# virajmehta/vae-training

Measured on AMD Instinct MI355X. Metric: ELBO train-step samples/sec, higher is better.
Workload: dtype f32; 1 GPU; M: linear-padding dd3 pad9 (D=12) L=20 linear enc/dec -tdv eps=-1 lr=1e-3 (seed_linpadding_expts.sh:1); batch_per_gpu=65536, global_batch=65536, data_dim=12, latent_dim=20, params=533, parallelism=dp1, grad_exchange=none, launch=direct library call x2395 steps (arguments marshalled once), input_batches=48

## Files before the change

### vae_training_amd/csrc/linear_moments.hip

```cpp
#include <stdlib.h>

#include <type_traits>

#include "comm_dev.h"
#include "rng_dev.h"
#include "vaek_internal.h"

namespace vaek {

using f32x4 = __attribute__((ext_vector_type(4))) float;
using d2 = __attribute__((ext_vector_type(2))) double;
typedef __attribute__((address_space(3))) void lds_void_t;
typedef const __attribute__((address_space(1))) void glb_void_t;

constexpr int LNT = 512, LNW = LNT / 64;
constexpr int kLinMaxPersist = 64;
constexpr int kLinCarry = 2, kLinSlots = kLinMaxPersist + kLinCarry;
struct LinWindow { int first, count; };
struct LinWindows { LinWindow stream, reduce, update; };
constexpr LinWindows lin_windows(int K, int j) {
    const int s0 = kLinMaxPersist * j, s1 = s0 + kLinMaxPersist < K ? s0 + kLinMaxPersist : K;
    const bool last = s1 == K;
    const int r0 = s0 >= 1 ? s0 - 1 : 0, u0 = s0 >= 2 ? s0 - 2 : 0;
    return LinWindows{{s0, s1 - s0}, {r0, (last ? K : s1 - 1) - r0}, {u0, (last ? K : s1 - 2) - u0}};
}
constexpr int lin_launches(int K) { return (K + kLinMaxPersist - 1) / kLinMaxPersist; }
constexpr bool lin_windows_ok(int K) {
    int s = 0, r = 0, u = 0;
    for (int j = 0; j < lin_launches(K); ++j) {
        const LinWindows w = lin_windows(K, j);
        if (w.stream.first != s || w.reduce.first != r || w.update.first != u) return false;
        if (w.stream.count < 1 || w.stream.count > kLinMaxPersist || w.reduce.count < 1 || w.update.count < 1) return false;
        s += w.stream.count; r += w.reduce.count; u += w.update.count;
        if (r > s || u > r || s - w.update.first > kLinSlots) return false;
    }
    return s == K && r == K && u == K;
}
static_assert(lin_windows_ok(1) && lin_windows_ok(2) && lin_windows_ok(64) && lin_windows_ok(65) && lin_windows_ok(66) && lin_windows_ok(128) &&
              lin_windows_ok(129) && lin_windows_ok(130) && lin_windows_ok(960), "launch windows of a vaek_train_steps call");
static_assert(lin_windows(64, 0).update.count == 64 && lin_windows(130, 1).update.first == 62 && lin_windows(130, 1).reduce.first == 63 &&
              lin_windows(130, 2).update.count == 4, "launch windows of a vaek_train_steps call");
constexpr int kLinReduceSets = 1;
constexpr int kLinReduceWgs = 24;

constexpr int kLinCommBanks = 4;
struct LinComm { unsigned long long* peer[kMaxWorld]; int world, rank, ng2; };

constexpr int kLinShards = 8, kLinShardStride = 32;
struct LinPtrs { const float* x[64]; const float* z1[64]; const float* z2[64]; };
struct LinArgs {
    int has_update, n_reduce, n_stream;
    int B, D, L, ntiles, T;
    const float* x; const float* z1; const float* z2; float* partial_out;
    const float* partial_in; double* M_out;
    const double* M_in;
    int persistent, n_steps, sets;
    int n_red, n_str, slot_upd, slot_red, slot_str;
    int d_red, d_str;
    float* partial_base; double* M_base;
    unsigned* cnt_stream; unsigned* cnt_reduce; unsigned* status;
    float* params; float* grads; float* m; float* v; int32_t* step_dev; float lr;
    float inv_bt, eps_cli, rows, rows_over_bt; int off_eps, P;
    float* loss_hist; long long loss_hist_cap;
    int stagger;
    LinComm comm;
};

#ifndef VAEK_LIN_ABL
#define VAEK_LIN_ABL 0
#endif
#ifdef VAEK_LIN_STAMPS
#ifdef VAEK_LIN_FOUR_BLOCK_TU
static __device__ unsigned long long* g_lin_stamp_buf = nullptr;
#else
__device__ unsigned long long* g_lin_stamp_buf = nullptr;
#endif
int lin_stamps_four(unsigned long long* buf);
#define LIN_STAMP(i)                                                                                         \
    do {                                                                                                     \
        if (VAEK_LIN_STAMPS == 2) break;          \
        __builtin_amdgcn_sched_barrier(0);                                                                   \
        unsigned long long _t;                                                                               \
        unsigned long long _r;                                                                               \
        asm volatile("s_waitcnt vmcnt(0) lgkmcnt(0)\n\ts_memtime %0\n\ts_memrealtime %1\n\ts_waitcnt lgkmcnt(0)" : "=s"(_t), "=s"(_r)::"memory"); \
        if (g_lin_stamp_buf && threadIdx.x == 0) { g_lin_stamp_buf[i] = _t; g_lin_stamp_buf[16 + (i)] = _r; } \
        __builtin_amdgcn_sched_barrier(0);                                                                   \
    } while (0)
#define LIN_NOW(v)                                                                                           \
    do {                                                                                                     \
        __builtin_amdgcn_sched_barrier(0);                                                                   \
        if (VAEK_LIN_STAMPS == 2) asm volatile("s_memrealtime %0\n\ts_waitcnt lgkmcnt(0)" : "=s"(v)::"memory");             \
        else asm volatile("s_waitcnt vmcnt(0) lgkmcnt(0)\n\ts_memrealtime %0\n\ts_waitcnt lgkmcnt(0)" : "=s"(v)::"memory"); \
        __builtin_amdgcn_sched_barrier(0);                                                                   \
    } while (0)
#define LIN_NOWQ(v)                                     \
    do {                                                                                                     \
        __builtin_amdgcn_sched_barrier(0);                                                                   \
        asm volatile("s_memrealtime %0\n\ts_waitcnt lgkmcnt(0)" : "=s"(v)::"memory");                        \
        __builtin_amdgcn_sched_barrier(0);                                                                   \
    } while (0)
#define LIN_PUT(i, v) do { if (g_lin_stamp_buf && threadIdx.x == 0) g_lin_stamp_buf[i] = (v); } while (0)
#define LIN_PUTMAX(i, v) do { if (g_lin_stamp_buf && threadIdx.x == 0) atomicMax(&g_lin_stamp_buf[i], (v)); } while (0)
#else
#define LIN_STAMP(i) do {} while (0)
#define LIN_NOW(v) do {} while (0)
#define LIN_NOWQ(v) do {} while (0)
#define LIN_PUT(i, v) do {} while (0)
#define LIN_PUTMAX(i, v) do {} while (0)
#endif

__device__ __forceinline__ void lin_glds16(const void* gsrc, void* lds_wave_base) {
    __builtin_amdgcn_global_load_lds((glb_void_t*)gsrc, (lds_void_t*)lds_wave_base, 16, 0, 0);
}
template <int N> __device__ __forceinline__ void lin_wait_vmcnt() { asm volatile("s_waitcnt vmcnt(%0)" ::"n"(N) : "memory"); }
__device__ __forceinline__ void lin_barrier() { asm volatile("s_waitcnt lgkmcnt(0)\n\ts_barrier" ::: "memory"); }
__device__ __forceinline__ void lin_wait_vmcnt_upto(int n) {
    switch (n) {
        case 1: lin_wait_vmcnt<1>(); break;   case 2: lin_wait_vmcnt<2>(); break;   case 3: lin_wait_vmcnt<3>(); break;
        case 4: lin_wait_vmcnt<4>(); break;   case 5: lin_wait_vmcnt<5>(); break;   case 6: lin_wait_vmcnt<6>(); break;
        case 7: lin_wait_vmcnt<7>(); break;   case 8: lin_wait_vmcnt<8>(); break;   case 9: lin_wait_vmcnt<9>(); break;
        case 10: lin_wait_vmcnt<10>(); break; case 11: lin_wait_vmcnt<11>(); break; case 12: lin_wait_vmcnt<12>(); break;
        case 13: lin_wait_vmcnt<13>(); break; case 14: lin_wait_vmcnt<14>(); break; case 15: lin_wait_vmcnt<15>(); break;
        case 16: lin_wait_vmcnt<16>(); break; case 17: lin_wait_vmcnt<17>(); break; case 18: lin_wait_vmcnt<18>(); break;
        case 19: lin_wait_vmcnt<19>(); break; case 20: lin_wait_vmcnt<20>(); break;
        default: lin_wait_vmcnt<0>(); break;
    }
}

__device__ __host__ constexpr int lin_blk(int NB, int b1, int b2) { return b1 * NB - b1 * (b1 - 1) / 2 + (b2 - b1); }

__device__ __forceinline__ void st_sc1(float* p, float v) { __hip_atomic_store(p, v, __ATOMIC_RELAXED, __HIP_MEMORY_SCOPE_AGENT); }
__device__ __forceinline__ void st_sc1(double* p, double v) { __hip_atomic_store(p, v, __ATOMIC_RELAXED, __HIP_MEMORY_SCOPE_AGENT); }
__device__ __forceinline__ float ld_sc1(const float* p) { return __hip_atomic_load(p, __ATOMIC_RELAXED, __HIP_MEMORY_SCOPE_AGENT); }
__device__ __forceinline__ double ld_sc1(const double* p) { return __hip_atomic_load(p, __ATOMIC_RELAXED, __HIP_MEMORY_SCOPE_AGENT); }

__device__ __forceinline__ void lin_wait_count(const unsigned* cnt, unsigned target, unsigned* status, unsigned tag) {
    if (threadIdx.x == 0) {
        unsigned spins = 0, seen;
        while ((seen = __hip_atomic_load(cnt, __ATOMIC_RELAXED, __HIP_MEMORY_SCOPE_AGENT)) < target) {
            __builtin_amdgcn_s_sleep(16);
            if ((++spins & 1023u) == 0) {
                if (__hip_atomic_load(status, __ATOMIC_RELAXED, __HIP_MEMORY_SCOPE_AGENT)) break;
                if (spins > (1u << 21)) {
                    unsigned expect = 0;
                    __hip_atomic_compare_exchange_strong(status, &expect, 0x80000000u | tag | (seen & 0xffffu), __ATOMIC_RELAXED,
                                                         __ATOMIC_RELAXED, __HIP_MEMORY_SCOPE_AGENT);
                    break;
                }
            }
        }
    }
    __syncthreads();
}

__device__ __forceinline__ void lin_wait_shards(const unsigned* cnt, unsigned target, unsigned* status, unsigned tag) {
    if (threadIdx.x == 0) {
        unsigned spins = 0, seen;
        for (;;) {
            unsigned v[kLinShards];
#pragma unroll
            for (int k = 0; k < kLinShards; ++k) v[k] = __hip_atomic_load(cnt + k * kLinShardStride, __ATOMIC_RELAXED, __HIP_MEMORY_SCOPE_AGENT);
            seen = 0;
#pragma unroll
            for (int k = 0; k < kLinShards; ++k) seen += v[k];
            if (seen >= target) break;
            __builtin_amdgcn_s_sleep(4);
            if ((++spins & 1023u) == 0) {
                if (__hip_atomic_load(status, __ATOMIC_RELAXED, __HIP_MEMORY_SCOPE_AGENT)) break;
                if (spins > (1u << 21)) {
                    unsigned expect = 0;
                    __hip_atomic_compare_exchange_strong(status, &expect, 0x80000000u | tag | (seen & 0xffffu), __ATOMIC_RELAXED,
                                                         __ATOMIC_RELAXED, __HIP_MEMORY_SCOPE_AGENT);
                    break;
                }
            }
        }
    }
    __syncthreads();
}

__device__ __forceinline__ double lin_sum_over_ranks(const LinComm& c, unsigned epoch, int o, double v, unsigned* status) {
    const unsigned long long bits = (unsigned long long)__double_as_longlong(v), tag = (unsigned long long)epoch << 32;
    const long long bank = (long long)(epoch & (kLinCommBanks - 1)) * c.world * c.ng2;
    for (int p = 0; p < c.world; ++p) {
        unsigned long long* q = c.peer[p] + bank + (long long)c.rank * c.ng2 + 2 * o;
        __hip_atomic_store(q, tag | (bits & 0xffffffffull), __ATOMIC_RELAXED, __HIP_MEMORY_SCOPE_SYSTEM);
        __hip_atomic_store(q + 1, tag | (bits >> 32), __ATOMIC_RELAXED, __HIP_MEMORY_SCOPE_SYSTEM);
    }
    const unsigned long long* own = c.peer[c.rank] + bank + 2 * o;
    double sum = 0.0;
    unsigned spins = 0;
    bool dead = false;
    for (int r = 0; r < c.world; ++r) {
        unsigned long long lo = 0, hi = 0;
// ... 435 lines not shown
            for (int d = 0; d < (DT ? DT : 32); ++d) if (DT || d < D) s += Wdd[l * D + d] * P1[d * NFP + f];
            G[e] = s;
        }
        for (int e = t; e < L * D; e += LNT) {
            const int l = e / D, d = e % D;
            double s = sd[l] * P1[d * NFP + l] + bed[l] * P1[d * NFP + fone];
#pragma unroll
            for (int dd = 0; dd < (DT ? DT : 32); ++dd) if (DT || dd < D) s += Wed[dd * L + l] * P1[d * NFP + L + dd];
            dwd[e] = s;
        }
        }
        __syncthreads();
        LIN_STAMP(4);
        double ssq = 0.0, musq = 0.0, z2r = 0.0, klc = 0.0;
        if constexpr (DT > 0 && LT > 0 && (DT % 2 == 0) && (LT % 2 == 0) && LT * (NFP / 2) <= LNT && LT * DT <= LNT / 2) {
            static_assert(DT * LT + LT + LT * DT + DT + LT + 1 + 3 <= LNT + 64, "wave 0 must own the scalar outputs");
            if (t < 64) {
                constexpr int NS = (LT * DT + 63) / 64, NM = (LT * (DT + 1) + 63) / 64;
                double wa[NS], da[NS], qw[NM], qs[NM], qd[NM], qm[NM];
#pragma unroll
                for (int j = 0; j < NS; ++j) { const int e = min(t + 64 * j, LT * DT - 1); wa[j] = Wdd[e]; da[j] = dwd[e]; }
#pragma unroll
                for (int j = 0; j < NM; ++j) {
                    const int e = min(t + 64 * j, LT * (DT + 1) - 1), l = e / (DT + 1), dd = e % (DT + 1), f = dd < DT ? LT + dd : fone;
                    qw[j] = dd < DT ? Wed[dd * LT + l] : bed[l]; qs[j] = SM[l * NFP + f]; qd[j] = sd[l]; qm[j] = Mf[l * NFP + f];
                }
                const int dq = min(t, DT - 1), lq = min(t, LT - 1);
                const double px = P1[dq * NFP + LT + dq], pz = P1[dq * NFP + LT + DT + dq], po = P1[dq * NFP + fone], bq = bdd[dq];
                const double lvq = lvd[lq], evq = elv[lq];
                __builtin_amdgcn_sched_barrier(0);
#pragma unroll
                for (int j = 0; j < NS; ++j) ssq += t + 64 * j < LT * DT ? wa[j] * da[j] : 0.0;
#pragma unroll
                for (int j = 0; j < NM; ++j) musq += t + 64 * j < LT * (DT + 1) ? qw[j] * (qs[j] - qd[j] * qm[j]) : 0.0;
                if (t < DT) { ssq += -px + sigma * pz + bq * po; z2r = pz; }
                if (t < LT) klc = 1.0 + lvq - evq;
#pragma unroll
                for (int o = 32; o > 0; o >>= 1) {
                    ssq += __shfl_xor(ssq, o, 64); musq += __shfl_xor(musq, o, 64);
                    z2r += __shfl_xor(z2r, o, 64); klc += __shfl_xor(klc, o, 64);
                }
            }
        } else {
        double p_ssq = 0.0, p_musq = 0.0, p_z2r = 0.0, p_klc = 0.0;
        for (int e = t; e < L * D; e += LNT) p_ssq += Wdd[e] * dwd[e];
        if (t < D) {
            p_ssq += -P1[t * NFP + L + t] + sigma * P1[t * NFP + L + D + t] + bdd[t] * P1[t * NFP + fone];
            p_z2r = P1[t * NFP + L + D + t];
        }
        for (int e = t; e < L * (D + 1); e += LNT) {
            const int l = e / (D + 1), dd = e % (D + 1);
            const int f = dd < D ? L + dd : fone;
            const double q = SM[l * NFP + f] - sd[l] * Mf[l * NFP + f];
            p_musq += (dd < D ? Wed[dd * L + l] : bed[l]) * q;
        }
        if (t < L) p_klc = 1.0 + lvd[t] - elv[t];
#pragma unroll
        for (int o = 32; o > 0; o >>= 1) {
            p_ssq += __shfl_xor(p_ssq, o, 64); p_musq += __shfl_xor(p_musq, o, 64);
            p_z2r += __shfl_xor(p_z2r, o, 64); p_klc += __shfl_xor(p_klc, o, 64);
        }
        if ((t & 63) == 0) { red[t >> 6] = p_ssq; red[LNW + (t >> 6)] = p_musq; red[2 * LNW + (t >> 6)] = p_z2r; red[3 * LNW + (t >> 6)] = p_klc; }
        __syncthreads();
#pragma unroll
        for (int w = 0; w < LNW; ++w) { ssq += red[w]; musq += red[LNW + w]; z2r += red[2 * LNW + w]; klc += red[3 * LNW + w]; }
        }
        LIN_STAMP(5);
        const double inv_bt = (double)a.inv_bt, rows = (double)a.rows, c0 = inv_var * inv_bt;
        const float bc1 = -expm1f((float)tstep * -0.10536051565782628f), bc2 = -expm1f((float)tstep * -0.0010005003335835335f);
#pragma unroll
        for (int k = 0; k < LKOUT; ++k) {
            const int idx = t + LNT * k;
            double gd = 0.0;
            if (idx < off_be) { const int d = idx / L, l = idx % L; gd = c0 * G[l * NFP + L + d] + (SM[l * NFP + L + d] - sd[l] * Mf[l * NFP + L + d]) * inv_bt; }
            else if (idx < off_wd) { const int l = idx - off_be; gd = c0 * G[l * NFP + fone] + (SM[l * NFP + fone] - sd[l] * Mf[l * NFP + fone]) * inv_bt; }
            else if (idx < off_bd) gd = c0 * dwd[idx - off_wd];
            else if (idx < off_epsp) gd = c0 * P1[(idx - off_bd) * NFP + fone];
            else if (idx < off_epsp + L) {
                const int l = idx - off_epsp;
                gd = 0.5 * sd[l] * c0 * G[l * NFP + l] - 0.5 * (1.0 - elv[l]) * (double)a.rows_over_bt;
            } else if (idx == off_eps) {
                gd = (double)a.eps_cli * (-0.5 * ssq * inv_var + 0.5 * rows * D + 0.5 * sigma * z2r * inv_var) * inv_bt;
            } else if (idx >= P && idx < P + 3) {
                const double dkl = (0.5 * musq - 0.5 * rows * klc) * inv_bt;
                const double mse = (0.5 * ssq * inv_var + 0.5 * rows * D * ((double)kLog2Pi + eps)) * inv_bt;
                gd = idx == P ? dkl + mse : (idx == P + 1 ? dkl : mse);
            }
            const float gf = (float)gd;
            gout[k] = gf;
            if (idx == P && a.loss_hist) a.loss_hist[(long long)(tstep - 1) % a.loss_hist_cap] = gf;
            if (idx < P) adam_apply_f(p[k], gf, m[k], v[k], a.lr, bc1, bc2);
        }
        LIN_STAMP(6);
    }
    __device__ __forceinline__ void store_state(const LinArgs& a, const float (&gout)[LKOUT], int tstep) {
        const int t = threadIdx.x;
#pragma unroll
        for (int k = 0; k < LKOUT; ++k) {
            const int idx = t + LNT * k;
            if (idx < P + kExtra) a.grads[idx] = gout[k];
            if (idx < P) { a.params[idx] = p[k]; a.m[idx] = m[k]; a.v[idx] = v[k]; }
        }
        if (t == 0) a.step_dev[0] = tstep;
    }
};

using d4 = __attribute__((ext_vector_type(4))) double;
template <int CTRL>
__device__ __forceinline__ double lin_dpp_add(double x) {
    const int lo = __builtin_amdgcn_update_dpp(0, __double2loint(x), CTRL, 0xf, 0xf, false);
    const int hi = __builtin_amdgcn_update_dpp(0, __double2hiint(x), CTRL, 0xf, 0xf, false);
    return x + __hiloint2double(hi, lo);
}
__device__ __forceinline__ double lin_wave_sum(double x) {
    x = lin_dpp_add<0xB1>(x);
    x = lin_dpp_add<0x4E>(x);
    x = lin_dpp_add<0x141>(x);
    x = lin_dpp_add<0x140>(x);
    double tot = 0.0;
#pragma unroll
    for (int r = 0; r < 4; ++r)
        tot += __hiloint2double(__builtin_amdgcn_readlane(__double2hiint(x), 16 * r), __builtin_amdgcn_readlane(__double2loint(x), 16 * r));
    return tot;
}
template <bool InLoop = false>
__device__ __forceinline__ double lin_exp(double x) {
    auto c = [](double v) __attribute__((always_inline)) { if constexpr (InLoop) asm volatile("" : "+s"(v)); return v; };
    const double k = rint(x * c(1.4426950408889634));
    double r = fma(-k, c(6.93147180369123816490e-01), x);
    r = fma(-k, c(1.90821492927058770002e-10), r);
    double p = c(1.0 / 6227020800.0);
    p = fma(p, r, c(1.0 / 479001600.0)); p = fma(p, r, c(1.0 / 39916800.0)); p = fma(p, r, c(1.0 / 3628800.0)); p = fma(p, r, c(1.0 / 362880.0));
    p = fma(p, r, c(1.0 / 40320.0)); p = fma(p, r, c(1.0 / 5040.0)); p = fma(p, r, c(1.0 / 720.0)); p = fma(p, r, c(1.0 / 120.0));
    p = fma(p, r, c(1.0 / 24.0)); p = fma(p, r, c(1.0 / 6.0)); p = fma(p, r, 0.5); p = fma(p, r, 1.0); p = fma(p, r, 1.0);
    return ldexp(p, (int)k);
}
__device__ __forceinline__ int lin_m_index(int NB, int r, int c) {
    const int br = r >> 4, bc = c >> 4;
    const int b1 = br <= bc ? br : bc, b2 = br <= bc ? bc : br, i = br <= bc ? (r & 15) : (c & 15), j = br <= bc ? (c & 15) : (r & 15);
    return lin_blk(NB, b1, b2) * 256 + (((i >> 2) * 16 + j) << 2) + (i & 3);
}
template <int NB, int DT, int LT>
struct LinUpdM {
    static constexpr int NFP = 16 * NB;
    static constexpr int KD = DT ? (DT + 3) / 4 : 4;
    static constexpr int RL1 = LT ? (LT > 16 ? (LT - 16 + 3) / 4 : 0) : 4;
    static constexpr int NM = 4 + RL1 + 2 * KD + 1;
    int D, L, P, fone, off_be, off_wd, off_bd, off_epsp, off_eps;
    double *Wed, *Wdd, *bed, *bdd, *sd, *elv, *lvd, *scal, *part, *P1s, *gq;
    float p[LKOUT], m[LKOUT], v[LKOUT];
    int mo[NM];

    static __host__ __device__ constexpr bool shape_ok(int D, int L) { return D <= 16 && L <= 32 && L + 2 * D + 1 <= NFP && NB == 3; }
    static __host__ size_t lds_bytes(int D, int L, int P) {
        return sizeof(double) * ((size_t)2 * D * L + 4 * L + D + 8 + 16 + 16 * NFP + (size_t)(P + kExtra + 7));
    }
    __device__ __forceinline__ void carve(const LinArgs& a, char* smem) {
        D = DT ? DT : a.D; L = LT ? LT : a.L; P = a.P; fone = L + 2 * D; off_eps = a.off_eps;
        off_be = D * L; off_wd = off_be + L; off_bd = off_wd + L * D; off_epsp = off_bd + D;
        Wed = reinterpret_cast<double*>(smem); Wdd = Wed + D * L; bed = Wdd + L * D; bdd = bed + L; sd = bdd + D; elv = sd + L; lvd = elv + L;
        scal = lvd + L; part = scal + 8; P1s = part + 16; gq = P1s + 16 * NFP;
    }
    __device__ __forceinline__ void load_state(const LinArgs& a) {
        const int t = threadIdx.x;
#pragma unroll
        for (int k = 0; k < LKOUT; ++k) {
            const int idx = min(t + LNT * k, P - 1);
            p[k] = a.params[idx]; m[k] = a.m[idx]; v[k] = a.v[idx];
        }
        if (off_eps < 0 && t == 0) { const double e = (double)a.eps_cli; scal[0] = e; scal[1] = lin_exp(0.5 * e); scal[2] = lin_exp(-e); }
        const int lane = t & 63, j = lane & 15, g = lane >> 4, f = min(16 * (t >> 6) + j, NFP - 1);
        int k = 0;
#pragma unroll
        for (int r = 0; r < 4; ++r) mo[k++] = lin_m_index(NB, g + 4 * r, f);
#pragma unroll
        for (int r = 0; r < RL1; ++r) mo[k++] = lin_m_index(NB, min(16 + g + 4 * r, NFP - 1), f);
#pragma unroll
        for (int r = 0; r < KD; ++r) mo[k++] = lin_m_index(NB, min(L + g + 4 * r, NFP - 1), f);
#pragma unroll
        for (int r = 0; r < KD; ++r) mo[k++] = lin_m_index(NB, min(L + D + g + 4 * r, NFP - 1), f);
        mo[k++] = lin_m_index(NB, fone, f);
    }
    __device__ __forceinline__ void fetch_M(const double* M_in, double (&r)[NM]) const {
#pragma unroll
        for (int k = 0; k < NM; ++k) r[k] = ld_sc1(M_in + mo[k]);
    }
    __device__ __forceinline__ void publish_params(const LinArgs& a) {
        const int t = threadIdx.x;
#pragma unroll
        for (int k = 0; k < LKOUT; ++k) {
            const int i = t + LNT * k;
            const double pv = (double)p[k];
            if (i < off_be) Wed[i] = pv;
            else if (i < off_wd) bed[i - off_be] = pv;
            else if (i < off_bd) Wdd[i - off_wd] = pv;
            else if (i < off_epsp) bdd[i - off_bd] = pv;
            else if (i < off_epsp + L || i == off_eps) {
                const bool is_eps = i == off_eps;
                const double e = is_eps ? pv * (double)a.eps_cli : pv, h = lin_exp(0.5 * e);
                if (is_eps) {
                    const double q = h * h;
                    double r = __builtin_amdgcn_rcp(q);
                    r = fma(fma(-q, r, 1.0), r, r); r = fma(fma(-q, r, 1.0), r, r);
                    scal[0] = e; scal[1] = h; scal[2] = r;
                }
                else { sd[i - off_epsp] = h; elv[i - off_epsp] = h * h; lvd[i - off_epsp] = pv; }
            }
        }
    }
    __device__ __forceinline__ void step(const LinArgs& a, int tstep, const double (&mreg)[NM], float (&gout)[LKOUT], const unsigned* next_cnt,
                                         unsigned per_set, const double* M_next, double (&mnext)[NM], bool& have_next) {
        const int t = threadIdx.x, wave = __builtin_amdgcn_readfirstlane(t >> 6), lane = t & 63, j = lane & 15, g = lane >> 4;
        LIN_STAMP(1);
        if (t == 64 * (NB + 2)) scal[4] = (next_cnt && __hip_atomic_load(next_cnt, __ATOMIC_RELAXED, __HIP_MEMORY_SCOPE_AGENT) >= per_set) ? 1.0 : 0.0;
        const double eps = scal[0], sigma = scal[1], inv_var = scal[2], inv_bt = (double)a.inv_bt, c0 = inv_var * inv_bt;
        d4 sm[2], p1;
        double musq_p = 0.0, ssq_p = 0.0, z2r_p = 0.0;
        const int f = 16 * wave + j;
        double awSMr[KD][2], awP1r[4 + (RL1 ? RL1 : 1)];
        auto awSM = [&](int kk, int lt) -> double& { return awSMr[kk][lt]; };
        auto awP1 = [&](int r) -> double& { return awP1r[r]; };
        if (wave < NB) {
#pragma unroll
            for (int kk = 0; kk < KD; ++kk)
#pragma unroll
                for (int lt = 0; lt < 2; ++lt) {
                    const int dd = 4 * kk + g, l = 16 * lt + j;
                    const double w1 = Wed[min(dd, D - 1) * L + min(l, L - 1)];
                    awSM(kk, lt) = (dd < D && l < L && (lt == 0 || RL1 > 0)) ? w1 : 0.0;
                }
#pragma unroll
            for (int r = 0; r < 4 + RL1; ++r) {
                const int l = (r < 4 ? 4 * r : 16 + 4 * (r - 4)) + g;
                const double w = Wdd[min(l, L - 1) * D + min(j, D - 1)];
                awP1(r) = (j < D && l < L) ? w : 0.0;
            }
        }
        __builtin_amdgcn_sched_barrier(0);
        if (wave < NB) {
            const double* Mz = mreg; const double* Mx = mreg + 4 + RL1; const double* Mz2 = Mx + KD; const double Mone = mreg[NM - 1];
#pragma unroll
            for (int lt = 0; lt < 2; ++lt)
#pragma unroll
                for (int r = 0; r < 4; ++r) {
                    const int l = 16 * lt + g + 4 * r;
                    const bool ok = l < L && (lt == 0 || r < RL1);
                    const double sv = sd[min(l, L - 1)], bv = bed[min(l, L - 1)];
                    const double slv = ok ? sv : 0.0, blv = ok ? bv : 0.0;
                    sm[lt][r] = (lt == 0 || r < RL1) ? slv * Mz[lt == 0 ? r : min(4 + r, 3 + RL1)] + blv * Mone : 0.0;
                }
#pragma unroll
            for (int kk = 0; kk < KD; ++kk) {
#pragma unroll
                for (int lt = 0; lt < 2; ++lt) {
                    if (lt == 1 && RL1 == 0) continue;
                    sm[lt] = __builtin_amdgcn_mfma_f64_16x16x4f64(awSM(kk, lt), Mx[kk], sm[lt], 0, 0, 0);
                }
            }
#pragma unroll
            for (int r = 0; r < 4; ++r) {
                const int d = g + 4 * r;
                p1[r] = (r < KD && d < D) ? -Mx[min(r, KD - 1)] + sigma * Mz2[min(r, KD - 1)] + bdd[min(d, D - 1)] * Mone : 0.0;
            }
#pragma unroll
            for (int r = 0; r < 4; ++r) p1 = __builtin_amdgcn_mfma_f64_16x16x4f64(awP1(r), sm[0][r], p1, 0, 0, 0);
#pragma unroll
            for (int r = 0; r < RL1; ++r) p1 = __builtin_amdgcn_mfma_f64_16x16x4f64(awP1(4 + r), sm[1][r], p1, 0, 0, 0);
#pragma unroll
            for (int r = 0; r < 4; ++r) P1s[(g + 4 * r) * NFP + f] = p1[r];
        } else if (wave == NB + 1) {
            const double kl = lane < L ? 1.0 + lvd[min(lane, L - 1)] - elv[min(lane, L - 1)] : 0.0;
            const double tot = lin_wave_sum(kl);
            if (lane == 0) {
                part[12] = tot;
                part[13] = (double)(-expm1f((float)tstep * -0.10536051565782628f)); part[14] = (double)(-expm1f((float)tstep * -0.0010005003335835335f));
            }
        }
        LIN_STAMP(2);
        __syncthreads();
        LIN_STAMP(3);
        have_next = scal[4] != 0.0;
        if (wave < NB) {
            if (have_next) fetch_M(M_next, mnext);
            double awGr[KD][2];
#pragma unroll
            for (int kk = 0; kk < KD; ++kk)
#pragma unroll
                for (int lt = 0; lt < 2; ++lt) {
                    const int dd = 4 * kk + g, l = 16 * lt + j;
                    const double w2 = Wdd[min(l, L - 1) * D + min(dd, D - 1)];
                    awGr[kk][lt] = (l < L && dd < D && (lt == 0 || RL1 > 0)) ? w2 : 0.0;
                }
            double sl[2][4], bl[2][4];
#pragma unroll
            for (int lt = 0; lt < 2; ++lt)
#pragma unroll
                for (int r = 0; r < 4; ++r) {
                    const int l = 16 * lt + g + 4 * r;
                    const bool ok = l < L && (lt == 0 || r < RL1);
                    const double sv = sd[min(l, L - 1)], bv = bed[min(l, L - 1)];
                    sl[lt][r] = ok ? sv : 0.0; bl[lt][r] = ok ? bv : 0.0;
                }
            __builtin_amdgcn_sched_barrier(0);
            d4 G[2];
            G[0] = d4{0.0, 0.0, 0.0, 0.0}; G[1] = d4{0.0, 0.0, 0.0, 0.0};
#pragma unroll
            for (int r = 0; r < KD; ++r) {
#pragma unroll
                for (int lt = 0; lt < 2; ++lt) {
                    if (lt == 1 && RL1 == 0) continue;
                    G[lt] = __builtin_amdgcn_mfma_f64_16x16x4f64(awGr[r][lt], p1[r], G[lt], 0, 0, 0);
                }
            }
            const double* Mz = mreg;
            const bool is_x = f >= L && f < L + D, is_z2 = f >= L + D && f < fone, is_one = f == fone, is_z1 = f < L;
            if (is_x || is_one) {
                const int base = is_x ? (f - L) * L : off_be;
#pragma unroll
                for (int lt = 0; lt < 2; ++lt)
#pragma unroll
                    for (int r = 0; r < 4; ++r) {
                        if (lt == 1 && r >= RL1) continue;
                        const int l = 16 * lt + g + 4 * r;
                        if (l < L) {
                            const double q = sm[lt][r] - sl[lt][r] * Mz[lt == 0 ? r : min(4 + r, 3 + RL1)];
                            gq[base + l] = c0 * G[lt][r] + q * inv_bt;
                            musq_p += (is_x ? Wed[base + l] : bl[lt][r]) * q;
                        }
                    }
            }
            if (is_one) {
#pragma unroll
                for (int r = 0; r < 4; ++r) {
                    const int d = g + 4 * r;
                    if (d < D) { gq[off_bd + d] = c0 * p1[r]; ssq_p += bdd[d] * p1[r]; }
                }
            }
            if (is_z1 && (j & 3) == g) {
                const int lt = f >> 4, r = j >> 2;
                double gll = 0.0;
#pragma unroll
                for (int q2 = 0; q2 < 2; ++q2)
#pragma unroll
                    for (int r2 = 0; r2 < 4; ++r2) gll = (q2 == lt && r2 == r) ? G[q2][r2] : gll;
                gq[off_epsp + f] = 0.5 * sd[f] * c0 * gll - 0.5 * (1.0 - elv[f]) * (double)a.rows_over_bt;
            }
            if (is_x || is_z2) {
                const int d = is_x ? f - L : f - L - D;
                if ((d & 3) == g) {
                    double pd = 0.0;
#pragma unroll
                    for (int r2 = 0; r2 < 4; ++r2) pd = (r2 == (d >> 2)) ? p1[r2] : pd;
                    if (is_x) ssq_p -= pd; else { ssq_p += sigma * pd; z2r_p += pd; }
                }
            }
            musq_p = lin_wave_sum(musq_p); ssq_p = lin_wave_sum(ssq_p); z2r_p = lin_wave_sum(z2r_p);
            if (lane == 0) { part[3 * wave] = ssq_p; part[3 * wave + 1] = musq_p; part[3 * wave + 2] = z2r_p; }
        } else if (wave == NB) {
            d4 C[2];
            double wsum = 0.0, avk[KD], p1l[2][4], p1o[4], dw_sr[2], dw_br[2], dw_wr[KD][2], dw_dr[2][4];
            auto dw_s = [&](int ct) -> double& { return dw_sr[ct]; };
            auto dw_b = [&](int ct) -> double& { return dw_br[ct]; };
            auto dw_w = [&](int kk, int ct) -> double& { return dw_wr[kk][ct]; };
            auto dw_d = [&](int ct, int r) -> double& { return dw_dr[ct][r]; };
#pragma unroll
            for (int ct = 0; ct < 2; ++ct) {
                const int l = 16 * ct + j, lc = min(l, L - 1);
                const double s_l = sd[lc], b_l = bed[lc];
                dw_s(ct) = l < L ? s_l : 0.0; dw_b(ct) = l < L ? b_l : 0.0;
#pragma unroll
                for (int kk = 0; kk < KD; ++kk) {
                    const int dd = 4 * kk + g;
                    const double w = Wed[min(dd, D - 1) * L + lc];
                    dw_w(kk, ct) = (dd < D && l < L) ? w : 0.0;
                }
#pragma unroll
                for (int r = 0; r < 4; ++r) dw_d(ct, r) = Wdd[lc * D + min(g + 4 * r, D - 1)];
            }
#pragma unroll
            for (int kk = 0; kk < KD; ++kk) avk[kk] = P1s[j * NFP + min(L + 4 * kk + g, NFP - 1)];
#pragma unroll
            for (int r = 0; r < 4; ++r) {
                p1o[r] = P1s[(g + 4 * r) * NFP + fone];
#pragma unroll
                for (int ct = 0; ct < 2; ++ct) p1l[ct][r] = P1s[(g + 4 * r) * NFP + min(16 * ct + j, L - 1)];
            }
            __builtin_amdgcn_sched_barrier(0);
#pragma unroll
            for (int ct = 0; ct < 2; ++ct) {
                if (ct == 1 && RL1 == 0) continue;
                const int l = 16 * ct + j;
#pragma unroll
                for (int r = 0; r < 4; ++r) C[ct][r] = dw_s(ct) * p1l[ct][r] + dw_b(ct) * p1o[r];
#pragma unroll
                for (int kk = 0; kk < KD; ++kk) C[ct] = __builtin_amdgcn_mfma_f64_16x16x4f64(avk[kk], dw_w(kk, ct), C[ct], 0, 0, 0);
#pragma unroll
                for (int r = 0; r < 4; ++r) {
                    const int d = g + 4 * r;
                    if (l < L && d < D) { gq[off_wd + l * D + d] = c0 * C[ct][r]; wsum += dw_d(ct, r) * C[ct][r]; }
                }
            }
            wsum = lin_wave_sum(wsum);
            if (lane == 0) part[9] = wsum;
        }
        LIN_STAMP(4);
        __syncthreads();
        LIN_STAMP(5);
        const double rows = (double)a.rows;
        const float bc1 = (float)part[13], bc2 = (float)part[14];
#pragma unroll
        for (int k = 0; k < LKOUT; ++k) {
            const int idx = t + LNT * k;
            if (LNT * k >= P + 3) break;
            double gd = 0.0;
            if (idx < P && idx != off_eps) gd = gq[idx];
            else if (idx == off_eps || (idx >= P && idx < P + 3)) {
                const double ssq = part[0] + part[3] + part[6] + part[9], musq = part[1] + part[4] + part[7], z2r = part[2] + part[5] + part[8], klc = part[12];
                if (idx == off_eps) gd = (double)a.eps_cli * (-0.5 * ssq * inv_var + 0.5 * rows * D + 0.5 * sigma * z2r * inv_var) * inv_bt;
                else {
                    const double dkl = (0.5 * musq - 0.5 * rows * klc) * inv_bt;
                    const double mse = (0.5 * ssq * inv_var + 0.5 * rows * D * ((double)kLog2Pi + eps)) * inv_bt;
                    gd = idx == P ? dkl + mse : (idx == P + 1 ? dkl : mse);
                }
            }
            const float gf = (float)gd;
            gout[k] = gf;
            if (idx == P && a.loss_hist) a.loss_hist[(long long)(tstep - 1) % a.loss_hist_cap] = gf;
            if (idx < P) adam_apply_f(p[k], gf, m[k], v[k], a.lr, bc1, bc2);
        }
        LIN_STAMP(6);
    }
    __device__ __forceinline__ void store_state(const LinArgs& a, const float (&gout)[LKOUT], int tstep) {
        const int t = threadIdx.x;
#pragma unroll
        for (int k = 0; k < LKOUT; ++k) {
            const int idx = t + LNT * k;
            if (idx < P + kExtra) a.grads[idx] = gout[k];
            if (idx < P) { a.params[idx] = p[k]; a.m[idx] = m[k]; a.v[idx] = v[k]; }
        }
        if (t == 0) a.step_dev[0] = tstep;
    }
};

template <int NB, int DT, int LT>
struct LinUpdMG {
    static constexpr int NFP = 16 * NB;
    static constexpr int KD = DT ? (DT + 3) / 4 : (NB == 3 ? 4 : 8);
    static constexpr int RL1 = LT ? (LT > 16 ? (LT - 16 + 3) / 4 : 0) : 4;
    static constexpr int NM = 4 + RL1 + 2 * KD + 1;
    static constexpr int PT = KD > 4 ? 2 : 1;
    static constexpr int NPART = NB == 3 ? 16 : 20;
    static constexpr bool PREFETCH = NB == 3;
    int D, L, P, fone, off_be, off_wd, off_bd, off_epsp, off_eps;
    double *Wed, *Wdd, *bed, *bdd, *sd, *elv, *lvd, *scal, *part, *P1s, *gq;
    float* pmv;
    __device__ __forceinline__ float& pk(int k) const { return pmv[k * LNT + threadIdx.x]; }
    __device__ __forceinline__ float& mk(int k) const { return pmv[(LKOUT + k) * LNT + threadIdx.x]; }
    __device__ __forceinline__ float& vk(int k) const { return pmv[(2 * LKOUT + k) * LNT + threadIdx.x]; }
    int* mos;

    static __host__ __device__ constexpr bool shape_ok(int D, int L) {
        return NB == 3 ? D <= 16 && L <= 32 && L + 2 * D + 1 <= NFP : NB == 4 && L <= 32 && L + 2 * D + 1 <= NFP && D <= 4 * KD;
    }
    static __host__ size_t lds_bytes(int D, int L, int P) {
        return sizeof(double) * ((size_t)2 * D * L + 4 * L + D + 8 + NPART + 16 * PT * NFP + (size_t)(P + kExtra + 7)) + sizeof(int) * NM * 64 * NB + sizeof(float) * 3 * LKOUT * LNT;
    }
    __device__ __forceinline__ void carve(const LinArgs& a, char* smem) {
        D = DT ? DT : a.D; L = LT ? LT : a.L; P = a.P; fone = L + 2 * D; off_eps = a.off_eps;
        off_be = D * L; off_wd = off_be + L; off_bd = off_wd + L * D; off_epsp = off_bd + D;
        Wed = reinterpret_cast<double*>(smem); Wdd = Wed + D * L; bed = Wdd + L * D; bdd = bed + L; sd = bdd + D; elv = sd + L; lvd = elv + L;
        scal = lvd + L; part = scal + 8; P1s = part + NPART; gq = P1s + 16 * PT * NFP; mos = reinterpret_cast<int*>(gq + P + kExtra + 7);
        pmv = reinterpret_cast<float*>(smem + sizeof(double) * (size_t)(gq + P + kExtra + 7 - Wed) + sizeof(int) * NM * 64 * NB);
    }
    __device__ __forceinline__ void load_state(const LinArgs& a) {
        const int t = threadIdx.x;
#pragma unroll
        for (int k = 0; k < LKOUT; ++k) {
            const int idx = min(t + LNT * k, P - 1);
            pk(k) = a.params[idx]; mk(k) = a.m[idx]; vk(k) = a.v[idx];
        }
        if (off_eps < 0 && t == 0) { const double e = (double)a.eps_cli; scal[0] = e; scal[1] = lin_exp<true>(0.5 * e); scal[2] = lin_exp<true>(-e); }
        if (t < 64 * NB) {
            const int lane = t & 63, j = lane & 15, g = lane >> 4, f = 16 * (t >> 6) + j;
            int k = 0;
            auto put = [&](int row) { mos[(k++) * 64 * NB + t] = lin_m_index(NB, row, f); };
#pragma unroll
            for (int r = 0; r < 4; ++r) put(g + 4 * r);
#pragma unroll
            for (int r = 0; r < RL1; ++r) put(min(16 + g + 4 * r, NFP - 1));
#pragma unroll
            for (int r = 0; r < KD; ++r) put(min(L + g + 4 * r, NFP - 1));
#pragma unroll
            for (int r = 0; r < KD; ++r) put(min(L + D + g + 4 * r, NFP - 1));
            put(fone);
        }
    }
    __device__ __forceinline__ void fetch_M(const double* M_in, double (&r)[NM]) const {
        const int* mt = mos + threadIdx.x;
        int o[NM];
#pragma unroll
        for (int k = 0; k < NM; ++k) o[k] = mt[k * 64 * NB];
#pragma unroll
        for (int k = 0; k < NM; ++k) r[k] = ld_sc1(M_in + o[k]);
    }
    __device__ __forceinline__ void publish_params(const LinArgs& a) {
        int t = threadIdx.x;
        if constexpr (NB == 4) asm volatile("" : "+v"(t));
#pragma unroll
        for (int k = 0; k < LKOUT; ++k) {
            const int i = t + LNT * k;
            const double pv = (double)pk(k);
            if (i < off_be) Wed[i] = pv;
            else if (i < off_wd) bed[i - off_be] = pv;
            else if (i < off_bd) Wdd[i - off_wd] = pv;
            else if (i < off_epsp) bdd[i - off_bd] = pv;
            else if (i < off_epsp + L || i == off_eps) {
                const bool is_eps = i == off_eps;
                const double e = is_eps ? pv * (double)a.eps_cli : pv, h = lin_exp<true>(0.5 * e);
                if (is_eps) {
                    const double q = h * h;
                    double r = __builtin_amdgcn_rcp(q);
                    r = fma(fma(-q, r, 1.0), r, r); r = fma(fma(-q, r, 1.0), r, r);
                    scal[0] = e; scal[1] = h; scal[2] = r;
                }
                else { sd[i - off_epsp] = h; elv[i - off_epsp] = h * h; lvd[i - off_epsp] = pv; }
            }
        }
    }
    __device__ __forceinline__ void step(const LinArgs& a, int tstep, const double (&mreg)[NM], float (&gout)[LKOUT], const unsigned* next_cnt,
                                         unsigned per_set, const double* M_next, double (&mnext)[NM], bool& have_next) {
        int t = threadIdx.x;
        if constexpr (NB == 4) asm volatile("" : "+v"(t));
        const int wave = __builtin_amdgcn_readfirstlane(t >> 6), lane = t & 63, j = lane & 15, g = lane >> 4;
        LIN_STAMP(1);
        if (PREFETCH && t == 64 * (NB + 2)) scal[4] = (next_cnt && __hip_atomic_load(next_cnt, __ATOMIC_RELAXED, __HIP_MEMORY_SCOPE_AGENT) >= per_set) ? 1.0 : 0.0;
        const double eps = scal[0], sigma = scal[1], inv_var = scal[2], inv_bt = (double)a.inv_bt, c0 = inv_var * inv_bt;
        d4 sm[2], p1;
        [[maybe_unused]] d4 p1b;
        auto p1row = [&](int r) -> double { return r < 4 ? p1[r & 3] : p1b[r & 3]; };
        double musq_p = 0.0, ssq_p = 0.0, z2r_p = 0.0;
        const int f = 16 * wave + j;
        double awSMr[KD][2], awP1r[PT][4 + (RL1 ? RL1 : 1)];
        auto awSM = [&](int kk, int lt) -> double& { return awSMr[kk][lt]; };
        auto awP1 = [&](int r) -> double& { return awP1r[0][r]; };
        if (wave < NB) {
#pragma unroll
            for (int kk = 0; kk < KD; ++kk)
#pragma unroll
                for (int lt = 0; lt < 2; ++lt) {
                    const int dd = 4 * kk + g, l = 16 * lt + j;
                    const double w1 = Wed[min(dd, D - 1) * L + min(l, L - 1)];
                    awSM(kk, lt) = (dd < D && l < L && (lt == 0 || RL1 > 0)) ? w1 : 0.0;
                }
#pragma unroll
            for (int r = 0; r < 4 + RL1; ++r) {
                const int l = (r < 4 ? 4 * r : 16 + 4 * (r - 4)) + g;
                const double w = Wdd[min(l, L - 1) * D + min(j, D - 1)];
                awP1(r) = (j < D && l < L) ? w : 0.0;
            }
        }
        __builtin_amdgcn_sched_barrier(0);
        if (wave < NB) {
            const double* Mz = mreg; const double* Mx = mreg + 4 + RL1; const double* Mz2 = Mx + KD; const double Mone = mreg[NM - 1];
#pragma unroll
            for (int lt = 0; lt < 2; ++lt)
#pragma unroll
                for (int r = 0; r < 4; ++r) {
                    const int l = 16 * lt + g + 4 * r;
                    const bool ok = l < L && (lt == 0 || r < RL1);
                    const double sv = sd[min(l, L - 1)], bv = bed[min(l, L - 1)];
                    const double slv = ok ? sv : 0.0, blv = ok ? bv : 0.0;
                    sm[lt][r] = (lt == 0 || r < RL1) ? slv * Mz[lt == 0 ? r : min(4 + r, 3 + RL1)] + blv * Mone : 0.0;
                }
#pragma unroll
            for (int kk = 0; kk < KD; ++kk) {
#pragma unroll
                for (int lt = 0; lt < 2; ++lt) {
                    if (lt == 1 && RL1 == 0) continue;
                    sm[lt] = __builtin_amdgcn_mfma_f64_16x16x4f64(awSM(kk, lt), Mx[kk], sm[lt], 0, 0, 0);
                }
            }
#pragma unroll
            for (int r = 0; r < 4; ++r) {
                const int d = g + 4 * r;
                p1[r] = (r < KD && d < D) ? -Mx[min(r, KD - 1)] + sigma * Mz2[min(r, KD - 1)] + bdd[min(d, D - 1)] * Mone : 0.0;
            }
#pragma unroll
            for (int r = 0; r < 4; ++r) p1 = __builtin_amdgcn_mfma_f64_16x16x4f64(awP1(r), sm[0][r], p1, 0, 0, 0);
#pragma unroll
            for (int r = 0; r < RL1; ++r) p1 = __builtin_amdgcn_mfma_f64_16x16x4f64(awP1(4 + r), sm[1][r], p1, 0, 0, 0);
#pragma unroll
// ... 812 lines not shown
```

Baseline: 18.86 billion samples/s.

## Deepen updater carry window and remap parameter slots for one exp per thread

Widens the slot carry between the streamer, reducer and updater windows from two to four batches, so the updater can trail further behind without stalling at launch boundaries. It also remaps which parameter each updater thread owns: the scalar outputs and eps go to a reserved wave, and overflow slots are assigned in reverse order. Because of this, each thread evaluates at most one exponential in publish_params, done after the loop, which shortens the serial critical path in the updater. The cost is more index arithmetic per slot and more slot buffer memory.

Result: faster. 19.23 billion samples/s (median of 6 runs) (+1.9%).

```diff
diff --git a/vae_training_amd/csrc/linear_moments.hip b/vae_training_amd/csrc/linear_moments.hip
--- a/vae_training_amd/csrc/linear_moments.hip
+++ b/vae_training_amd/csrc/linear_moments.hip
@@ -15,14 +15,15 @@
 
 constexpr int LNT = 512, LNW = LNT / 64;
 constexpr int kLinMaxPersist = 64;
-constexpr int kLinCarry = 2, kLinSlots = kLinMaxPersist + kLinCarry;
+constexpr int kLinCarry = 4, kLinSlots = kLinMaxPersist + kLinCarry;
+static_assert(kLinCarry >= 2 && kLinCarry < kLinMaxPersist, "the updater follows the reducers, which follow the streamers by one batch");
 struct LinWindow { int first, count; };
 struct LinWindows { LinWindow stream, reduce, update; };
 constexpr LinWindows lin_windows(int K, int j) {
     const int s0 = kLinMaxPersist * j, s1 = s0 + kLinMaxPersist < K ? s0 + kLinMaxPersist : K;
     const bool last = s1 == K;
-    const int r0 = s0 >= 1 ? s0 - 1 : 0, u0 = s0 >= 2 ? s0 - 2 : 0;
-    return LinWindows{{s0, s1 - s0}, {r0, (last ? K : s1 - 1) - r0}, {u0, (last ? K : s1 - 2) - u0}};
+    const int r0 = s0 >= 1 ? s0 - 1 : 0, u0 = s0 >= kLinCarry ? s0 - kLinCarry : 0;
+    return LinWindows{{s0, s1 - s0}, {r0, (last ? K : s1 - 1) - r0}, {u0, (last ? K : s1 - kLinCarry) - u0}};
 }
 constexpr int lin_launches(int K) { return (K + kLinMaxPersist - 1) / kLinMaxPersist; }
 constexpr bool lin_windows_ok(int K) {
@@ -37,9 +38,10 @@
     return s == K && r == K && u == K;
 }
 static_assert(lin_windows_ok(1) && lin_windows_ok(2) && lin_windows_ok(64) && lin_windows_ok(65) && lin_windows_ok(66) && lin_windows_ok(128) &&
-              lin_windows_ok(129) && lin_windows_ok(130) && lin_windows_ok(960), "launch windows of a vaek_train_steps call");
-static_assert(lin_windows(64, 0).update.count == 64 && lin_windows(130, 1).update.first == 62 && lin_windows(130, 1).reduce.first == 63 &&
-              lin_windows(130, 2).update.count == 4, "launch windows of a vaek_train_steps call");
+              lin_windows_ok(129) && lin_windows_ok(130) && lin_windows_ok(132) && lin_windows_ok(960), "launch windows of a vaek_train_steps call");
+static_assert(lin_windows(64, 0).update.count == 64 && lin_windows(130, 1).update.first == 64 - kLinCarry && lin_windows(130, 1).reduce.first == 63 &&
+              lin_windows(130, 2).update.count == 2 + kLinCarry && lin_windows(65, 0).update.count == 64 - kLinCarry &&
+              lin_windows(65, 1).update.count == 1 + kLinCarry, "launch windows of a vaek_train_steps call");
 constexpr int kLinReduceSets = 1;
 constexpr int kLinReduceWgs = 24;
 
@@ -781,6 +783,24 @@
     int mo[NM];
 
     static __host__ __device__ constexpr bool shape_ok(int D, int L) { return D <= 16 && L <= 32 && L + 2 * D + 1 <= NFP && NB == 3; }
+    static constexpr int kSpecT0 = LNT - 64, kOvfTop = kSpecT0 - 1;
+    static_assert(LNT - (kExtra + 1) - kOvfTop > 32 && kOvfTop + 1 > 32, "publish_params: one exponential per thread needs two slots of a thread more than L <= 32 outputs apart");
+    __device__ __forceinline__ int out_index(int t, int k) const {
+        const int ns = kExtra + (off_eps >= 0 ? 1 : 0), np = P - (off_eps >= 0 ? 1 : 0);
+        int r;
+        if (k == 0) {
+            if (t >= kSpecT0 && t < kSpecT0 + ns) return t - kSpecT0 < kExtra ? P + (t - kSpecT0) : off_eps;
+            r = t < kSpecT0 ? t : t - ns;
+        } else {
+            if (t > kOvfTop) return -1;
+            r = LNT - ns + (kOvfTop + 1) * (k - 1) + (kOvfTop - t);
+        }
+        if (r >= np) return -1;
+        return r + ((off_eps >= 0 && r >= off_eps) ? 1 : 0);
+    }
+    __device__ __forceinline__ bool slot_used(int k) const {
+        return k == 0 || LNT - (kExtra + (off_eps >= 0 ? 1 : 0)) + (kOvfTop + 1) * (k - 1) < P - (off_eps >= 0 ? 1 : 0);
+    }
     static __host__ size_t lds_bytes(int D, int L, int P) {
         return sizeof(double) * ((size_t)2 * D * L + 4 * L + D + 8 + 16 + 16 * NFP + (size_t)(P + kExtra + 7));
     }
@@ -794,7 +814,7 @@
         const int t = threadIdx.x;
 #pragma unroll
         for (int k = 0; k < LKOUT; ++k) {
-            const int idx = min(t + LNT * k, P - 1);
+            const int o = out_index(t, k), idx = o >= 0 && o < P ? o : P - 1;
             p[k] = a.params[idx]; m[k] = a.m[idx]; v[k] = a.v[idx];
         }
         if (off_eps < 0 && t == 0) { const double e = (double)a.eps_cli; scal[0] = e; scal[1] = lin_exp(0.5 * e); scal[2] = lin_exp(-e); }
@@ -816,25 +836,30 @@
     }
     __device__ __forceinline__ void publish_params(const LinArgs& a) {
         const int t = threadIdx.x;
+        int ei = -1;
+        double epv = 0.0;
 #pragma unroll
         for (int k = 0; k < LKOUT; ++k) {
-            const int i = t + LNT * k;
+            if (!slot_used(k)) break;
+            const int i = out_index(t, k);
             const double pv = (double)p[k];
+            if (i < 0 || i >= P) continue;
             if (i < off_be) Wed[i] = pv;
             else if (i < off_wd) bed[i - off_be] = pv;
             else if (i < off_bd) Wdd[i - off_wd] = pv;
             else if (i < off_epsp) bdd[i - off_bd] = pv;
-            else if (i < off_epsp + L || i == off_eps) {
-                const bool is_eps = i == off_eps;
-                const double e = is_eps ? pv * (double)a.eps_cli : pv, h = lin_exp(0.5 * e);
-                if (is_eps) {
-                    const double q = h * h;
-                    double r = __builtin_amdgcn_rcp(q);
-                    r = fma(fma(-q, r, 1.0), r, r); r = fma(fma(-q, r, 1.0), r, r);
-                    scal[0] = e; scal[1] = h; scal[2] = r;
-                }
-                else { sd[i - off_epsp] = h; elv[i - off_epsp] = h * h; lvd[i - off_epsp] = pv; }
-            }
+            else if (i < off_epsp + L || i == off_eps) { ei = i; epv = pv; }
+        }
+        if (ei >= 0) {
+            const bool is_eps = ei == off_eps;
+            const double e = is_eps ? epv * (double)a.eps_cli : epv, h = lin_exp<true>(0.5 * e);
+            if (is_eps) {
+                const double q = h * h;
+                double r = __builtin_amdgcn_rcp(q);
+                r = fma(fma(-q, r, 1.0), r, r); r = fma(fma(-q, r, 1.0), r, r);
+                scal[0] = e; scal[1] = h; scal[2] = r;
+            }
+            else { sd[ei - off_epsp] = h; elv[ei - off_epsp] = h * h; lvd[ei - off_epsp] = epv; }
         }
     }
     __device__ __forceinline__ void step(const LinArgs& a, int tstep, const double (&mreg)[NM], float (&gout)[LKOUT], const unsigned* next_cnt,
@@ -1039,11 +1064,11 @@
         const float bc1 = (float)part[13], bc2 = (float)part[14];
 #pragma unroll
         for (int k = 0; k < LKOUT; ++k) {
-            const int idx = t + LNT * k;
-            if (LNT * k >= P + 3) break;
+            if (!slot_used(k)) break;
+            const int idx = out_index(t, k);
             double gd = 0.0;
-            if (idx < P && idx != off_eps) gd = gq[idx];
-            else if (idx == off_eps || (idx >= P && idx < P + 3)) {
+            if (idx >= 0 && idx < P && idx != off_eps) gd = gq[idx];
+            else if (k == 0 && idx >= 0 && (idx == off_eps || (idx >= P && idx < P + 3))) {
                 const double ssq = part[0] + part[3] + part[6] + part[9], musq = part[1] + part[4] + part[7], z2r = part[2] + part[5] + part[8], klc = part[12];
                 if (idx == off_eps) gd = (double)a.eps_cli * (-0.5 * ssq * inv_var + 0.5 * rows * D + 0.5 * sigma * z2r * inv_var) * inv_bt;
                 else {
@@ -1055,7 +1080,7 @@
             const float gf = (float)gd;
             gout[k] = gf;
             if (idx == P && a.loss_hist) a.loss_hist[(long long)(tstep - 1) % a.loss_hist_cap] = gf;
-            if (idx < P) adam_apply_f(p[k], gf, m[k], v[k], a.lr, bc1, bc2);
+            if (idx >= 0 && idx < P) adam_apply_f(p[k], gf, m[k], v[k], a.lr, bc1, bc2);
         }
         LIN_STAMP(6);
     }
@@ -1063,9 +1088,9 @@
         const int t = threadIdx.x;
 #pragma unroll
         for (int k = 0; k < LKOUT; ++k) {
-            const int idx = t + LNT * k;
-            if (idx < P + kExtra) a.grads[idx] = gout[k];
-            if (idx < P) { a.params[idx] = p[k]; a.m[idx] = m[k]; a.v[idx] = v[k]; }
+            const int idx = out_index(t, k);
+            if (idx >= 0 && idx < P + kExtra) a.grads[idx] = gout[k];
+            if (idx >= 0 && idx < P) { a.params[idx] = p[k]; a.m[idx] = m[k]; a.v[idx] = v[k]; }
         }
         if (t == 0) a.step_dev[0] = tstep;
     }
```
